# bendalab/audian

Hardware: AMD Instinct MI355X
Metric: Msamples/s spectrogram+bandpass, 64ch x 96kHz (higher is better)
Workload: dtype f32 I/O, f64 IIR state; 1 GPU; BASELINE configs[2]: synthetic 64 ch/GPU x 600 s x 96 kHz float32; bandpass 300-3000 Hz order 2 -> spectrogram nfft 2048 hop 1024 + envelope 20 Hz; channels_per_gpu=64, frames=57600000, spectrogram_frames=56250, parallelism=channel shard x1, streams=one compute stream, envelope_forward=state checkpoints, fused into the band-pass kernel, envelope_buffer=best of 4 allocations by memset time (hipdsp_malloc_probed), spectrogram=FFT waves inside the forward sweep (filtered tiles from LDS)

## Files before the change

### audian_amd/csrc/sos.hip

```cpp
#include "sos_device.h"
#include <cmath>
#include <vector>

namespace {
template <int S>
__global__ __launch_bounds__(64 * WPB) void sos_scan_kernel(const SosPlanDev *__restrict__ P0, SeqArgs a)
{
    constexpr int D = 2 * S;
    __shared__ float4 lds_all[WPB][64 * 8];
    const int wave = __builtin_amdgcn_readfirstlane(threadIdx.x >> 6);
    float4 *lds = lds_all[wave];
    const int lane = threadIdx.x & 63;
    const long long unit = (long long)blockIdx.x * WPB + wave;
    if (unit >= a.units) return;
    const int seg = (int)(unit % a.n_seg);
    const long long ch = unit / a.n_seg;
    const float *in = a.in + ch * a.in_pitch;
    float *out = a.out + ch * a.out_pitch;

    const long long lo = (long long)seg * a.seg_len;
    long long hi = lo + a.seg_len;
    if (hi > a.N) hi = a.N;
    long long start = lo - P0->warm;
    if (start < 0) start = 0;
// ... 260 lines not shown
    constexpr int D = 2 * SE;
    double *ckpt = ckpt_all + (long long)blockIdx.x * ckpt_pitch;
    flood_channel(flood, blockIdx.x);
    {
        __shared__ int any_bad;
        if (threadIdx.x == 0) any_bad = 0;
        __syncthreads();
        for (long long j = first_seg + threadIdx.x; j < n_seg; j += blockDim.x) {
            const double *e = ckpt + (j + 1 < n_seg ? (j + 1) * seg_tiles : n_tiles) * D;
            bool bad = false;
#pragma unroll
            for (int r = 0; r < D; r++) bad = bad || !(fabs(e[r]) <= 1.7976931348623157e308);
            if (bad) atomicOr(&any_bad, 1);
        }
        __syncthreads();
        if (any_bad && threadIdx.x == 0) ckpt[n_tiles * D] = __builtin_nan("");
        __syncthreads();
    }
    double AT[D][D];
#pragma unroll
    for (int r = 0; r < D; r++)
#pragma unroll
        for (int c = 0; c < D; c++) AT[r][c] = P0->AT[r * D + c];
    const long long warm_tiles = P0->warm / TILE;
    const long long terms = (warm_tiles + seg_tiles - 1) / seg_tiles + 1;
    const long long steps = seg_tiles <= warm_tiles ? seg_tiles : 0;
    for (long long k_hi = n_seg - 1; k_hi >= first_seg + 1; k_hi -= blockDim.x) {
        const long long k = k_hi - threadIdx.x;
        double S[D];
#pragma unroll
        for (int r = 0; r < D; r++) S[r] = 0.0;
        if (k >= first_seg + 1) {
            long long j = k - terms;
            if (j < first_seg) j = first_seg;
            for (; j < k; j++) {
                const double *e = ckpt + (j + 1) * seg_tiles * D;
                if (steps == 0) {
#pragma unroll
                    for (int r = 0; r < D; r++) S[r] = 0.0;
                }
                for (long long m = 0; m < steps; m++) {
                    double t[D];
#pragma unroll
                    for (int r = 0; r < D; r++) {
                        double acc = 0.0;
#pragma unroll
                        for (int c = 0; c < D; c++) acc = fma(AT[r][c], S[c], acc);
                        t[r] = acc;
                    }
#pragma unroll
                    for (int r = 0; r < D; r++) S[r] = t[r];
                }
#pragma unroll
                for (int r = 0; r < D; r++) S[r] += e[r];
            }
        }
        __syncthreads();
        if (k >= first_seg + 1) {
            const long long t0 = k * seg_tiles;
            long long cnt = (k == n_seg - 1) ? n_tiles - t0 : seg_tiles;
            if (cnt > warm_tiles + 1) cnt = warm_tiles + 1;
#pragma unroll
            for (int r = 0; r < D; r++) ckpt[t0 * D + r] = S[r];
            for (long long m = 1; m < cnt; m++) {
                double t[D];
#pragma unroll
                for (int r = 0; r < D; r++) {
                    double acc = 0.0;
#pragma unroll
                    for (int c = 0; c < D; c++) acc = fma(AT[r][c], S[c], acc);
                    t[r] = acc;
                }
#pragma unroll
                for (int r = 0; r < D; r++) { S[r] = t[r]; ckpt[(t0 + m) * D + r] += t[r]; }
            }
        }
        __syncthreads();
    }
}

int launch_env_fix(hipdsp_ctx *ctx, const SosPlanDev *edev, int SE, double *ckpt, long long ckpt_pitch, long long channels,
                   int n_seg, long long seg_len, long long n_tiles, const FloodArgs *flood, int first_seg = 0)
{
    if (n_seg <= 1) return HIPDSP_OK;
    dim3 grid((unsigned)channels), block(256);
    const long long seg_tiles = seg_len / TILE;
    FloodArgs fl;
    memset(&fl, 0, sizeof(fl));
    if (flood) fl = *flood;
    switch (SE) {
    case 1: hipLaunchKernelGGL((env_fix_kernel<1>), grid, block, 0, ctx->stream, edev, ckpt, ckpt_pitch, n_seg, seg_tiles, n_tiles, fl, first_seg); break;
    case 2: hipLaunchKernelGGL((env_fix_kernel<2>), grid, block, 0, ctx->stream, edev, ckpt, ckpt_pitch, n_seg, seg_tiles, n_tiles, fl, first_seg); break;
    case 3: hipLaunchKernelGGL((env_fix_kernel<3>), grid, block, 0, ctx->stream, edev, ckpt, ckpt_pitch, n_seg, seg_tiles, n_tiles, fl, first_seg); break;
    case 4: hipLaunchKernelGGL((env_fix_kernel<4>), grid, block, 0, ctx->stream, edev, ckpt, ckpt_pitch, n_seg, seg_tiles, n_tiles, fl, first_seg); break;
    default: return HIPDSP_OK;
    }
    return hd_launch_status("env_fix_kernel");
}

template <int SE, bool PREFETCH, bool PIN = true, bool TRACE = false, int WPB_ = WPB, bool REGW = (SE <= 2)>
__global__ __launch_bounds__(64 * WPB_, REGW ? 2 : 1) void env_bwd_kernel(const SosPlanDev *__restrict__ P0, BwdArgs a)
{
    long long tr_acc[6] = {0, 0, 0, 0, 0, 0};
    long long tr_last = TRACE ? clock64() : 0;
#define TRACE_AT(i)                                              \
    do {                                                         \
        if (TRACE) {                                             \
            const long long t_ = clock64();                      \
            tr_acc[(i)] += t_ - tr_last;                         \
            tr_last = t_;                                        \
        }                                                        \
    } while (0)
    constexpr int DE = 2 * SE;
    __shared__ float4 lds_all[WPB_][64 * 8];
    const int wave = __builtin_amdgcn_readfirstlane(threadIdx.x >> 6);
    float4 *lds = lds_all[wave];
    float *ldsf = reinterpret_cast<float *>(lds);
    const int lane = threadIdx.x & 63;
    const long long unit = (long long)blockIdx.x * WPB_ + wave;
    if (unit >= a.units) return;
    const int seg = (int)(unit % a.n_seg);
    const long long ch = unit / a.n_seg;
    const float *in = a.in + ch * a.in_pitch;
    float *out = a.out + ch * a.out_pitch;
    const double *ckpt = a.ckpt + ch * a.ckpt_pitch;
    const long long T = a.T;
    const int edge = a.edge;
    const long long trace_t0 = a.trace ? wall_clock64() : 0;
    const unsigned slot = wave_slot_of_simd();

    const long long rt_lo = (long long)seg * a.seg_tiles;
    long long rt_hi = rt_lo + a.seg_tiles;
    if (rt_hi > a.n_tiles) rt_hi = a.n_tiles;
    long long rt_start = rt_lo - a.warm_tiles;
    if (rt_start < 0) rt_start = 0;

    double cb_[DE];
#pragma unroll
    for (int r = 0; r < DE; r++) cb_[r] = 0.0;

    {
        double end_state[DE];
#pragma unroll
        for (int r = 0; r < DE; r++) end_state[r] = ckpt[a.n_tiles * DE + r];
        if (state_not_finite(end_state)) {
            long long p_lo = (a.n_tiles - rt_hi) * TILE, p_hi = (a.n_tiles - rt_lo) * TILE;
            if (p_lo < a.skip) p_lo = a.skip;
            if (p_hi > T) p_hi = T;
            for (long long p = p_lo + lane; p < p_hi; p += 64) out[p - a.skip] = __builtin_nanf("");
            return;
        }
    }

    v4f nx[8], nck[SE];
    bool pre = false;
    auto fetch = [&](long long tidx) {
        const long long tsrc = (a.debug & 2) ? 0 : tidx;
#pragma unroll
        for (int k = 0; k < 8; k++) nx[k] = asm_load16(in + tsrc * TILE + 256 * k + 4 * lane);
#pragma unroll
        for (int i = 0; i < SE; i++) nck[i] = asm_load16(ckpt + tidx * DE + 2 * i);
    };
    const long long top_full = T / TILE - 1;
    auto prefetchable = [&](long long tidx) {
        return tidx >= 0 && tidx <= top_full && tidx * TILE + TILE > a.skip && tidx * TILE >= a.lead;
    };
    const long long env_tile0 = a.env0 > 0 ? a.env0 - a.env0 % TILE : -1;
    if (PREFETCH) {
        const long long t0 = a.n_tiles - 1 - rt_start;
        pre = rt_start < rt_hi && prefetchable(t0);
        fetch(pre ? t0 : top_full);
        asm volatile("s_waitcnt vmcnt(0)" ::: "memory");
    }

    for (long long rt = rt_start; rt < rt_hi; rt++) {
        const long long tidx = a.n_tiles - 1 - rt;
        const long long tile = tidx * TILE;
        if (tile + TILE <= a.skip) break;
        if (a.fair) rotate_issue_priority(slot);
        double cfw_[DE];
        if (PREFETCH && pre) {
            if (a.rectify) {
#pragma unroll
                for (int k = 0; k < 8; k++) {
                    asm volatile("" : "+v"(nx[k]));
                    lds[lds_slot(8 * k + (lane >> 3), lane & 7)] =
                        make_float4(fabsf(nx[k].x), fabsf(nx[k].y), fabsf(nx[k].z), fabsf(nx[k].w));
                }
            } else {
#pragma unroll
                for (int k = 0; k < 8; k++) {
                    asm volatile("" : "+v"(nx[k]));
                    lds[lds_slot(8 * k + (lane >> 3), lane & 7)] = make_float4(nx[k].x, nx[k].y, nx[k].z, nx[k].w);
                }
            }
#pragma unroll
            for (int i = 0; i < SE; i++) {
                asm volatile("" : "+v"(nck[i]));
                const v2d d = __builtin_bit_cast(v2d, nck[i]);
                cfw_[2 * i] = d.x; cfw_[2 * i + 1] = d.y;
            }
            WAVE_SYNC();
        } else if (PREFETCH) {
            const long long lead = a.lead;
#pragma unroll 1
            for (int k = 0; k < 8; k++) {
                const long long p = tile + 256 * k + 4 * lane;
                auto at = [&](long long q) { return in + (q < lead ? lead : (q < T ? q : T - 1)); };
                auto ok = [&](long long q) { return q >= lead && q < T; };
                v4f t;
                t.x = asm_load4(at(p));
                t.y = asm_load4(at(p + 1));
                t.z = asm_load4(at(p + 2));
                t.w = asm_load4(at(p + 3));
                asm volatile("s_waitcnt vmcnt(0)" ::: "memory");
                asm volatile("" : "+v"(t));
                float4 v = make_float4(ok(p) ? t.x : 0.f, ok(p + 1) ? t.y : 0.f, ok(p + 2) ? t.z : 0.f,
                                       ok(p + 3) ? t.w : 0.f);
                if (a.rectify) v = make_float4(fabsf(v.x), fabsf(v.y), fabsf(v.z), fabsf(v.w));
                lds[lds_slot(8 * k + (lane >> 3), lane & 7)] = v;
            }
            v4f ck[SE];
#pragma unroll
            for (int i = 0; i < SE; i++) ck[i] = asm_load16(ckpt + tidx * DE + 2 * i);
            float ra = asm_load4(in + (T - 1));
            float rb = asm_load4(in + (lane < edge ? T - 2 - lane : T - 1));
            asm volatile("s_waitcnt vmcnt(0)" ::: "memory");
#pragma unroll
            for (int i = 0; i < SE; i++) {
                asm volatile("" : "+v"(ck[i]));
                const v2d d = __builtin_bit_cast(v2d, ck[i]);
                cfw_[2 * i] = d.x; cfw_[2 * i + 1] = d.y;
            }
            asm volatile("" : "+v"(ra));
            asm volatile("" : "+v"(rb));
            WAVE_SYNC();
            if (lane < edge) {
                const long long pj = T + lane;
                if (pj >= tile && pj < tile + TILE) {
                    if (a.rectify) { ra = fabsf(ra); rb = fabsf(rb); }
                    ldsf[lds_float_index((int)(pj - tile))] = 2.f * ra - rb;
                }
            }
        } else {
#pragma unroll
            for (int k = 0; k < 8; k++) {
                float4 v = load_four_from(in, tile + 256 * k + 4 * lane, a.lead, T);
                if (a.rectify) v = make_float4(fabsf(v.x), fabsf(v.y), fabsf(v.z), fabsf(v.w));
                lds[lds_slot(8 * k + (lane >> 3), lane & 7)] = v;
            }
#pragma unroll
            for (int r = 0; r < DE; r++) cfw_[r] = ckpt[tidx * DE + r];
        }
        WAVE_SYNC();
        if (!PREFETCH && tile + TILE > T) {
            if (lane < edge) {
                const long long pj = T + lane;
                if (pj >= tile && pj < tile + TILE) {
                    float ra = in[T - 1], rb = in[T - 2 - lane];
                    if (a.rectify) { ra = fabsf(ra); rb = fabsf(rb); }
                    ldsf[lds_float_index((int)(pj - tile))] = 2.f * ra - rb;
                }
            }
            WAVE_SYNC();
        }
        if (PREFETCH) WAVE_SYNC();
        if (tile == env_tile0) {
            (void)env_left_fill(ldsf, lane, (int)(a.env0 - tile), edge);
        }
        TRACE_AT(0);
        if (PREFETCH) {
            pre = rt + 1 < rt_hi && prefetchable(tidx - 1);
            fetch(pre ? tidx - 1 : top_full);
        }
        TRACE_AT(1);
#define CASC_S SE
#define CASC_PLAN() PLAN_OF(P0)
#define CASC_IN(v) (v)
#define CASC_PIN_GROUPS PIN
      if constexpr (REGW) {
#define CASC_CARRY_AFTER_F
        double w_[L];
#define CASC_CARRY cfw_
#define CASC_GAIN a.gain
#define CASC_NO_STORE
#define CASC_TAP(j, e, y) w_[(j)] = (y)
#include "sos_cascade.inc"
#undef CASC_TAP
#undef CASC_NO_STORE
#undef CASC_GAIN
#undef CASC_CARRY
        WAVE_SYNC();
        TRACE_AT(2);
        if (rt == 0) {
            int last = (int)(T + edge - 1 - tile);
            asm volatile("" : "+v"(last));
            const int lrow = last >> 5, lj = last & 31;
            double v0 = 0.0;
#pragma unroll
            for (int j = 0; j < L; j++) v0 = (j == lj) ? w_[j] : v0;
            v0 = __shfl(v0, lrow, 64);
#pragma unroll
            for (int j = 0; j < L; j++) w_[j] = (L * lane + j > last) ? v0 : w_[j];
            const SosPlanDev *P = PLAN_OF(P0);
#pragma unroll
            for (int r = 0; r < DE; r++) cb_[r] = P->zi[r] * v0;
        }
#define CASC_CARRY cb_
#define CASC_DOWN
#define CASC_X(j) w_[L - 1 - (j)]
#include "sos_cascade.inc"
#undef CASC_X
#undef CASC_DOWN
#undef CASC_CARRY
#undef CASC_CARRY_AFTER_F
      } else {
#define CASC_CARRY cfw_
#define CASC_GAIN a.gain
#include "sos_cascade.inc"
#undef CASC_GAIN
#undef CASC_CARRY
        WAVE_SYNC();
        TRACE_AT(2);
        if (rt == 0) {
            const int last = (int)(T + edge - 1 - tile);
            const float v0 = ldsf[lds_float_index(last)];
            WAVE_SYNC();
            for (int s2 = last + 1 + lane; s2 < TILE; s2 += 64) ldsf[lds_float_index(s2)] = v0;
            const SosPlanDev *P = PLAN_OF(P0);
#pragma unroll
            for (int r = 0; r < DE; r++) cb_[r] = P->zi[r] * (double)v0;
            WAVE_SYNC();
        }
#define CASC_CARRY cb_
#define CASC_REVERSED
#include "sos_cascade.inc"
#undef CASC_REVERSED
#undef CASC_CARRY
      }
#undef CASC_PIN_GROUPS
#undef CASC_S
#undef CASC_PLAN
#undef CASC_IN
        WAVE_SYNC();
        TRACE_AT(3);
        if (rt >= rt_lo) {
            if (tile >= a.skip && tile + TILE <= T) {
                v4f rows[8];
                tile_rows_from_lds(lds, lane, rows);
                if (a.clamp) {
                    const long long tdst = (a.debug & 1) ? a.skip : tile;
#pragma unroll
                    for (int k = 0; k < 8; k++) {
                        const v4f v = rows[k];
                        f4u t; t.x = max_zero(v.x); t.y = max_zero(v.y); t.z = max_zero(v.z); t.w = max_zero(v.w);
                        *reinterpret_cast<f4u *>(out + (tdst + 256 * k + 4 * lane - a.skip)) = t;
                    }
                } else {
#pragma unroll
                    for (int k = 0; k < 8; k++) {
                        const v4f v = rows[k];
                        f4u t; t.x = v.x; t.y = v.y; t.z = v.z; t.w = v.w;
                        *reinterpret_cast<f4u *>(out + (tile + 256 * k + 4 * lane - a.skip)) = t;
                    }
                }
                TRACE_AT(4);
                if (PREFETCH) asm volatile("s_waitcnt vmcnt(7)" ::: "memory");
            } else {
#pragma unroll
                for (int k = 0; k < 8; k++) {
                    float4 v = lds[lds_slot(8 * k + (lane >> 3), lane & 7)];
                    if (a.clamp) {
                        v.x = fmaxf(v.x, 0.f); v.y = fmaxf(v.y, 0.f); v.z = fmaxf(v.z, 0.f); v.w = fmaxf(v.w, 0.f);
                    }
                    store_four(out, tile + 256 * k + 4 * lane, v, a.skip, T, a.skip);
                }
                if (PREFETCH) asm volatile("s_waitcnt vmcnt(0)" ::: "memory");
            }
        } else if (PREFETCH) {
            asm volatile("s_waitcnt vmcnt(0)" ::: "memory");
        }
        WAVE_SYNC();
        TRACE_AT(5);
    }
#undef TRACE_AT
    if (a.trace && lane == 0 && unit < a.trace_rows) {
        unsigned hw;
        asm volatile("s_getreg_b32 %0, hwreg(HW_REG_HW_ID)" : "=s"(hw));
        long long *tr = a.trace + 9 * unit;
        tr[0] = trace_t0;
        tr[1] = wall_clock64();
        tr[2] = hw;
#pragma unroll
        for (int i = 0; i < 6; i++) tr[3 + i] = tr_acc[i];
    }
}

__global__ __launch_bounds__(256) void odd_ext_kernel(const float *__restrict__ x, long long x_pitch, long long T, int edge, int rectify,
                                                      float *__restrict__ out, long long out_pitch)
{
    const long long ch = blockIdx.y;
    const float *xc = x + ch * x_pitch;
    float *oc = out + ch * out_pitch;
    const long long N = T + 2LL * edge;
    auto r = [&](long long k) { const float v = xc[k]; return rectify ? fabsf(v) : v; };
    const long long i = 4 * ((long long)blockIdx.x * 256 + threadIdx.x);
    if (i >= N) return;
    if (i >= edge && i + 4 <= edge + T) {
        f4u v = *reinterpret_cast<const f4u *>(xc + (i - edge));
        if (rectify) { v.x = fabsf(v.x); v.y = fabsf(v.y); v.z = fabsf(v.z); v.w = fabsf(v.w); }
        *reinterpret_cast<f4u *>(oc + i) = v;
        return;
    }
    for (long long j = i; j < i + 4 && j < N; j++) {
        float v;
        if (j < edge) v = 2.f * r(0) - r(edge - j);
        else if (j < edge + T) v = r(j - edge);
        else v = 2.f * r(T - 1) - r(T - 2 - (j - edge - T));
        oc[j] = v;
    }
}

__global__ __launch_bounds__(256) void flip_kernel(const float *__restrict__ x, long long x_pitch, long long N, long long first, long long n,
                                                   int clamp, float *__restrict__ y, long long y_pitch)
{
    const long long ch = blockIdx.y;
    const float *xc = x + ch * x_pitch;
    float *yc = y + ch * y_pitch;
    auto cl = [&](float v) { return (clamp && v < 0.f) ? 0.f : v; };
    const long long i = 4 * ((long long)blockIdx.x * 256 + threadIdx.x);
    if (i >= n) return;
    if (i + 4 <= n) {
        const f4u v = *reinterpret_cast<const f4u *>(xc + (N - 1 - (first + i) - 3));
        f4u o; o.x = cl(v.w); o.y = cl(v.z); o.z = cl(v.y); o.w = cl(v.x);
        *reinterpret_cast<f4u *>(yc + i) = o;
        return;
    }
    for (long long j = i; j < n; j++) yc[j] = cl(xc[N - 1 - (first + j)]);
}

__global__ void first_sample_kernel(const float *__restrict__ x, long long x_pitch, long long channels, float *__restrict__ ref)
{
    const long long c = (long long)blockIdx.x * blockDim.x + threadIdx.x;
    if (c < channels) ref[c] = x[c * x_pitch];
}

__global__ __launch_bounds__(256) void copy_skip_kernel(const float *__restrict__ x, long long x_pitch, float *__restrict__ y,
                                                        long long y_pitch, long long n, long long skip)
{
    const long long ch = blockIdx.y;
    const float *xi = x + ch * x_pitch + skip;
    float *yo = y + ch * y_pitch;
    const long long n4 = n / 4;
    const long long i = (long long)blockIdx.x * 256 + threadIdx.x;
    if (i < n4) {
        *reinterpret_cast<f4u *>(yo + 4 * i) = *reinterpret_cast<const f4u *>(xi + 4 * i);
    } else if (i == n4) {
        for (long long k = 4 * n4; k < n; k++) yo[k] = xi[k];
    }
}

int launch_scan(hipdsp_ctx *ctx, const SosPlanDev *dev, int S, SeqArgs a, long long channels, long long warm)
{
    if (a.gain == 0.0) a.gain = 1.0;
    plan_segments(ctx, a.N, channels, warm, &a.seg_len, &a.n_seg, -1);
    a.units = channels * a.n_seg;
    long long blocks = (a.units + WPB - 1) / WPB;
// ... 418 lines not shown
```

### audian_amd/csrc/sos_cascade.inc

```
#ifndef CASC_PIN_GROUPS
#define CASC_PIN_GROUPS false
#define CASC_PIN_DEFAULTED
#endif
#ifndef CASC_STAMP
#define CASC_STAMP(n)
#define CASC_STAMP_DEFAULTED
#endif
#ifndef CASC_UNIT_OK
#define CASC_UNIT_OK true
#define CASC_UNIT_DEFAULTED
#endif
#ifdef CASC_REVERSED
#define CASC_ROW (63 - lane)
#define CASC_Q(q) (7 - (q))
#define CASC_E(k) (3 - (k))
#elif defined(CASC_DOWN)
#define CASC_ROW lane
#define CASC_Q(q) (7 - (q))
#define CASC_E(k) (3 - (k))
#else
#define CASC_ROW lane
#define CASC_Q(q) (q)
#define CASC_E(k) (k)
#endif
#ifdef CASC_DOWN
#define CASC_SHIFT1(x) casc_wave_shl1(x)
#define CASC_SHIFT32(x) casc_wave_shl32(x)
#define CASC_SHIFT(x, d) __shfl_down((x), (d), 64)
#define CASC_FED(d) (lane < 64 - (d))
#define CASC_HEAD (lane == 63)
#define CASC_LAST 0
#else
#define CASC_SHIFT1(x) casc_wave_shr1(x)
#define CASC_SHIFT32(x) casc_wave_shr32(x)
#define CASC_SHIFT(x, d) __shfl_up((x), (d), 64)
#define CASC_FED(d) (lane >= (d))
#define CASC_HEAD (lane == 0)
#define CASC_LAST 63
#endif
#ifdef CASC_X
#define CASC_XD(q, k) (CASC_X(4 * (q) + (k)))
#else
#define CASC_XD(q, k) ((double)CASC_IN(e[CASC_E(k)]))
#endif
{
    constexpr int CD = 2 * CASC_S;
        double f[CD];
#ifdef CASC_F_IN
#pragma unroll
        for (int r = 0; r < CD; r++) f[r] = CASC_F_IN[r];
#else
#pragma unroll
        for (int r = 0; r < CD; r++) f[r] = 0.0;
        constexpr int GQ = CD <= 2 ? 4 : (CD <= 4 ? 2 : 1);
#ifdef CASC_ROLLED_GROUPS
#pragma unroll 1
#else
#pragma unroll
#endif
        for (int q0 = 0; q0 < 8; q0 += GQ) {
            const SosPlanDev *P = CASC_PLAN();
            double gg[GQ * 4 * CD];
            if (CASC_PIN_GROUPS) {
#pragma unroll
                for (int i = 0; i < GQ * 4 * CD; i++) gg[i] = P->G[4 * q0 * CD + i];
#pragma unroll
                for (int i = 0; i < GQ * 4 * CD; i++) asm volatile("" : "+s"(gg[i]));
            }
#define CASC_G(q, k, r) ((CASC_PIN_GROUPS) ? gg[(4 * ((q) - q0) + (k)) * CD + (r)] : P->G[(4 * (q) + (k)) * CD + (r)])
#pragma unroll
            for (int q = q0; q < q0 + GQ; q++) {
#ifndef CASC_X
                const float4 v = lds[lds_slot(CASC_ROW, CASC_Q(q))];
                const float e[4] = {v.x, v.y, v.z, v.w};
#endif
#pragma unroll
                for (int k = 0; k < 4; k++) {
                    const double xd = CASC_XD(q, k);
#pragma unroll
                    for (int r = 0; r < CD; r++) f[r] = fma(CASC_G(q, k, r), xd, f[r]);
                }
            }
#undef CASC_G
#ifdef CASC_X
            __builtin_amdgcn_sched_barrier(0);
#endif
        }
#ifdef CASC_GAIN
#pragma unroll
        for (int r = 0; r < CD; r++) f[r] *= (CASC_GAIN);
#endif
#endif
        CASC_STAMP(0);
        {
#ifdef CASC_CARRY_AFTER_F
#pragma unroll
            for (int r = 0; r < CD; r++) asm volatile("" : "+v"(f[r]), "+v"(CASC_CARRY[r]));
#endif
            const SosPlanDev *P = CASC_PLAN();
            double t[CD];
#pragma unroll
            for (int r = 0; r < CD; r++) {
                double acc = 0.0;
#pragma unroll
                for (int c = 0; c < CD; c++)
                    if (c / 2 <= r / 2) acc = fma(P->M[r * CD + c], CASC_CARRY[c], acc);
                t[r] = acc;
            }
#pragma unroll
            for (int r = 0; r < CD; r++) f[r] += CASC_HEAD ? t[r] : 0.0;
        }
        constexpr int GK = CD <= 2 ? 6 : (CD <= 4 ? 2 : 1);
#pragma unroll
        for (int k0 = 0; k0 < 6; k0 += GK) {
            const SosPlanDev *P = CASC_PLAN();
            double mm[GK * CD * CD];
            if (CASC_PIN_GROUPS) {
#pragma unroll
                for (int i = 0; i < GK * CD * CD; i++) mm[i] = P->M[k0 * CD * CD + i];
#pragma unroll
                for (int i = 0; i < GK * CD * CD; i++)
                    if ((i % CD) / 2 <= ((i / CD) % CD) / 2) asm volatile("" : "+s"(mm[i]));
            }
#define CASC_M(k, r, c) ((CASC_PIN_GROUPS) ? mm[((k) - k0) * CD * CD + (r) * CD + (c)] : P->M[(k) * CD * CD + (r) * CD + (c)])
#pragma unroll
            for (int k = k0; k < k0 + GK; k++) {
                const int d = 1 << k;
                double q[CD];
#pragma unroll
                for (int c = 0; c < CD; c++) {
                    if (k == 0) {
                        q[c] = CASC_SHIFT1(f[c]);
                    } else if (k == 5) {
                        q[c] = CASC_SHIFT32(f[c]);
                    } else {
                        q[c] = CASC_SHIFT(f[c], d);
                    }
                }
                if (k == 0 || k == 5 || CASC_FED(d)) {
#pragma unroll
                    for (int r = 0; r < CD; r++) {
                        double acc = f[r];
#pragma unroll
                        for (int c = 0; c < CD; c++)
                            if (c / 2 <= r / 2) acc = fma(CASC_M(k, r, c), q[c], acc);
                        f[r] = acc;
                    }
                }
            }
#undef CASC_M
        }
        CASC_STAMP(1);
#ifdef CASC_NO_OUTPUT
#pragma unroll
        for (int r = 0; r < CD; r++) CASC_CARRY[r] = __shfl(f[r], CASC_LAST, 64);
#else
        double z[CD];
#pragma unroll
        for (int r = 0; r < CD; r++) {
            const double s = CASC_SHIFT1(f[r]);
            z[r] = CASC_HEAD ? CASC_CARRY[r] : s;
        }
#pragma unroll
        for (int r = 0; r < CD; r++) CASC_CARRY[r] = __shfl(f[r], CASC_LAST, 64);

        {
            const SosPlanDev *P = CASC_PLAN();
            double cf[CASC_S][5];
#pragma unroll
            for (int s = 0; s < CASC_S; s++)
#pragma unroll
                for (int k = 0; k < 5; k++) cf[s][k] = P->coef[s][k];
#ifdef CASC_GAIN
#pragma unroll
            for (int k = 0; k < 3; k++) cf[0][k] *= (CASC_GAIN);
#endif
#define CASC_PHASE3(UNIT)                                                                         \
            _Pragma("unroll")                                                                      \
            for (int q = 0; q < 8; q++) {                                                          \
                CASC_PHASE3_LOAD(q)                                                                \
                _Pragma("unroll")                                                                  \
                for (int k = 0; k < 4; k++) {                                                      \
                    double cur = CASC_XD(q, k);                                                    \
                    _Pragma("unroll")                                                              \
                    for (int s = 0; s < CASC_S; s++) {                                             \
                        if ((UNIT) && s > 0) {                                                     \
                            const double y = cur + z[2 * s];                                       \
                            z[2 * s] = fma(-cf[s][3], y, fma(cf[s][1], cur, z[2 * s + 1]));        \
                            z[2 * s + 1] = fma(-cf[s][4], y, cur);                                 \
                            cur = y;                                                               \
                        } else {                                                                   \
                            const double y = fma(cf[s][0], cur, z[2 * s]);                         \
                            z[2 * s] = fma(-cf[s][3], y, fma(cf[s][1], cur, z[2 * s + 1]));        \
                            z[2 * s + 1] = fma(-cf[s][4], y, cf[s][2] * cur);                      \
                            cur = y;                                                               \
                        }                                                                          \
                    }                                                                              \
                    CASC_PHASE3_OUT(q, k)                                                          \
                }                                                                                  \
                CASC_PHASE3_STORE(q)                                                               \
            }
#ifdef CASC_X
#define CASC_PHASE3_LOAD(q) float e[4] = {0.f, 0.f, 0.f, 0.f};
#else
#define CASC_PHASE3_LOAD(q) const float4 v = lds[lds_slot(CASC_ROW, CASC_Q(q))]; float e[4] = {v.x, v.y, v.z, v.w};
#endif
#ifndef CASC_NO_STORE
#define CASC_PHASE3_SET(k) e[CASC_E(k)] = (float)cur;
#define CASC_PHASE3_STORE(q) lds[lds_slot(CASC_ROW, CASC_Q(q))] = make_float4(e[0], e[1], e[2], e[3]);
#else
#define CASC_PHASE3_SET(k)
#define CASC_PHASE3_STORE(q)
#endif
#ifdef CASC_TAP
#define CASC_PHASE3_OUT(q, k) CASC_PHASE3_SET(k) CASC_TAP((4 * (q) + (k)), e[CASC_E(k)], cur);
#else
#define CASC_PHASE3_OUT(q, k) CASC_PHASE3_SET(k)
#endif
            if (CASC_S > 1 && (CASC_UNIT_OK) && P->unit_tail != 0) {
                CASC_PHASE3(true)
            } else {
                CASC_PHASE3(false)
            }
#undef CASC_PHASE3
#undef CASC_PHASE3_LOAD
#undef CASC_PHASE3_SET
#undef CASC_PHASE3_STORE
#undef CASC_PHASE3_OUT
        }
        CASC_STAMP(2);
#endif
}
#ifdef CASC_STAMP_DEFAULTED
#undef CASC_STAMP
#undef CASC_STAMP_DEFAULTED
#endif
#ifdef CASC_UNIT_DEFAULTED
#undef CASC_UNIT_OK
#undef CASC_UNIT_DEFAULTED
#endif
#ifdef CASC_PIN_DEFAULTED
#undef CASC_PIN_GROUPS
#undef CASC_PIN_DEFAULTED
#endif
#undef CASC_ROW
#undef CASC_Q
#undef CASC_E
#undef CASC_SHIFT1
#undef CASC_SHIFT32
#undef CASC_SHIFT
#undef CASC_FED
#undef CASC_HEAD
#undef CASC_LAST
#undef CASC_XD
```

### audian_amd/csrc/sos_device.h

```cpp
#pragma once
#include "common.h"
#include "sos_plan.h"

struct hipdsp_sosplan {
    SosPlanDev *host;
    SosPlanDev *dev;
    hipEvent_t uploaded;
    bool valid;
};

struct FloodArgs {
    const unsigned char *flags;
    int n_seg;
    long long seg_len;
    float *y;
    long long y_pitch, T, skip;
    float *psd, *db;
    long long psd_pitch, n_valid;
    int F, nfft, hop;
    int frame_off;
};

int hd_launch_env_fix(hipdsp_ctx *ctx, const SosPlanDev *edev, int SE, double *ckpt, long long ckpt_pitch, long long channels,
                      int n_seg, long long seg_len, long long n_tiles, const FloodArgs *flood, int first_seg = 0);

struct BwdArgs {
    const float *in;
    float *out;
    const double *ckpt;
    long long in_pitch, out_pitch, ckpt_pitch;
    long long T, skip;
    long long n_tiles;
    long long seg_tiles, warm_tiles;
    int n_seg, edge, rectify, clamp;
    double gain;
    long long units;
    long long lead, env0;
    long long *trace;
    long long trace_rows;
    int debug;
    int fair;
};

namespace {


typedef float f4u __attribute__((ext_vector_type(4), aligned(4)));
typedef float f2u __attribute__((ext_vector_type(2), aligned(4)));

struct SeqArgs {
    const float *in;
    float *out;
    long long in_pitch, out_pitch;
    long long N;
    long long seg_len;
    int n_seg;
    long long skip;
    const float *zi_ref;
    long long zi_ref_pitch;
    double zi_scale;
    double gain;
    long long units;
    unsigned char *flags;
};

__device__ __forceinline__ long long opaque_zero()
{
    int z;
    asm volatile("s_mov_b32 %0, 0" : "=s"(z));
    return (long long)z;
}

__device__ __forceinline__ int lds_slot(int row, int q) { return row * 8 + (q ^ ((row & 7) ^ ((row >> 3) & 1))); }
__device__ __forceinline__ int lds_float_index(int s) { return lds_slot(s >> 5, (s & 31) >> 2) * 4 + (s & 3); }

__device__ __forceinline__ float4 load_four(const float *in, long long p, long long n)
{
    if (p + 4 <= n) {
        const f4u t = *reinterpret_cast<const f4u *>(in + p);
        return make_float4(t.x, t.y, t.z, t.w);
    }
    float4 v;
    v.x = p < n ? in[p] : 0.f;
    v.y = p + 1 < n ? in[p + 1] : 0.f;
    v.z = p + 2 < n ? in[p + 2] : 0.f;
    v.w = p + 3 < n ? in[p + 3] : 0.f;
    return v;
}

__device__ __forceinline__ float4 load_four_from(const float *in, long long p, long long first, long long n)
{
    if (p >= first) return load_four(in, p, n);
    float4 v;
    v.x = 0.f;
    v.y = (p + 1 >= first && p + 1 < n) ? in[p + 1] : 0.f;
    v.z = (p + 2 >= first && p + 2 < n) ? in[p + 2] : 0.f;
    v.w = (p + 3 >= first && p + 3 < n) ? in[p + 3] : 0.f;
    return v;
}

__device__ __forceinline__ void store_four(float *out, long long p, float4 v, long long lo, long long hi,
                                           long long shift)
{
    if (p >= lo && p + 4 <= hi) {
        f4u t; t.x = v.x; t.y = v.y; t.z = v.z; t.w = v.w;
        *reinterpret_cast<f4u *>(out + (p - shift)) = t;
    } else {
        const float e[4] = {v.x, v.y, v.z, v.w};
#pragma unroll
        for (int k = 0; k < 4; k++)
            if (p + k >= lo && p + k < hi) out[p + k - shift] = e[k];
    }
}

#define PLAN_OF(ptr) (reinterpret_cast<const SosPlanDev *>(reinterpret_cast<const char *>(ptr) + opaque_zero()))

__device__ __forceinline__ double casc_wave_shr1(double x)
{
    const long long b = __builtin_bit_cast(long long, x);
    const int lo = __builtin_amdgcn_update_dpp(0, (int)b, 0x138, 0xf, 0xf, true);
    const int hi = __builtin_amdgcn_update_dpp(0, (int)(b >> 32), 0x138, 0xf, 0xf, true);
    return __builtin_bit_cast(double, ((long long)hi << 32) | (unsigned int)lo);
}

__device__ __forceinline__ double casc_wave_shr32(double x)
{
    const long long b = __builtin_bit_cast(long long, x);
    const auto lo = __builtin_amdgcn_permlane32_swap(0, (int)b, false, false);
    const auto hi = __builtin_amdgcn_permlane32_swap(0, (int)(b >> 32), false, false);
    return __builtin_bit_cast(double, ((long long)hi[0] << 32) | (unsigned int)lo[0]);
}

__device__ __forceinline__ double casc_wave_shl1(double x)
{
    const long long b = __builtin_bit_cast(long long, x);
    const int lo = __builtin_amdgcn_update_dpp(0, (int)b, 0x130, 0xf, 0xf, true);
    const int hi = __builtin_amdgcn_update_dpp(0, (int)(b >> 32), 0x130, 0xf, 0xf, true);
    return __builtin_bit_cast(double, ((long long)hi << 32) | (unsigned int)lo);
}
__device__ __forceinline__ double casc_wave_shl32(double x)
{
    const long long b = __builtin_bit_cast(long long, x);
    const auto lo = __builtin_amdgcn_permlane32_swap((int)b, 0, false, false);
    const auto hi = __builtin_amdgcn_permlane32_swap((int)(b >> 32), 0, false, false);
    return __builtin_bit_cast(double, ((long long)hi[1] << 32) | (unsigned int)lo[1]);
}

#define WAVE_SYNC()                                          \
    do {                                                     \
        __builtin_amdgcn_fence(__ATOMIC_ACQ_REL, "wavefront"); \
        __builtin_amdgcn_wave_barrier();                     \
    } while (0)

constexpr int WPB = 4;

struct CkptArgs {
    const float *in;
    float *yf;
    double *ckpt;
    long long in_pitch, yf_pitch, ckpt_pitch;
    long long T, seg_len;
    int n_seg, edge, rectify;
    long long units;
    double gain;
    unsigned char *flags;
    long long lead;
    long long env0;
};

struct GridShift {
    long long lead, env0;
    int frame_off;
};
inline GridShift hd_grid_shift(long long spec_first, long long env_first, int hop, int edge, bool with_env)
{
    GridShift g;
    const long long step = hop > 0 ? hop : 128;
    g.lead = hop > 0 ? (step - spec_first % step) % step : 0;
    if (with_env && env_first + g.lead > 0) {
        for (int tries = 0; tries < 4; tries++) {
            const long long r = (env_first + g.lead) % TILE;
            if (r >= edge && r + edge < TILE) break;
            g.lead += step;
        }
    }
    g.env0 = with_env ? env_first + g.lead : 0;
    g.frame_off = hop > 0 ? (int)((spec_first + g.lead) / step) : 0;
    return g;
}

typedef float v4f __attribute__((ext_vector_type(4)));
__device__ __forceinline__ void tile_rows_from_lds(const float4 *lds, int lane, v4f (&v)[8])
{
#pragma unroll
    for (int k = 0; k < 8; k++) {
        const float4 t = lds[lds_slot(8 * k + (lane >> 3), lane & 7)];
        v[k] = (v4f){t.x, t.y, t.z, t.w};
    }
    asm volatile("" : "+v"(v[0]), "+v"(v[1]), "+v"(v[2]), "+v"(v[3]), "+v"(v[4]), "+v"(v[5]), "+v"(v[6]), "+v"(v[7]));
}
typedef double v2d __attribute__((ext_vector_type(2)));
__device__ __forceinline__ v4f asm_load16(const void *p)
{
    v4f r;
    asm volatile("global_load_dwordx4 %0, %1, off" : "=v"(r) : "v"(p) : "memory");
    return r;
}
__device__ __forceinline__ float asm_load4(const float *p)
{
    float r;
    asm volatile("global_load_dword %0, %1, off" : "=v"(r) : "v"(p) : "memory");
    return r;
}

__device__ __forceinline__ void rotate_issue_priority(unsigned slot)
{
    const unsigned p = (slot + (unsigned)(__builtin_readcyclecounter() >> 14)) & 3u;
    if (p == 0) __builtin_amdgcn_s_setprio(0);
    else if (p == 1) __builtin_amdgcn_s_setprio(1);
    else if (p == 2) __builtin_amdgcn_s_setprio(2);
    else __builtin_amdgcn_s_setprio(3);
}
__device__ __forceinline__ float max_zero(float x)
{
    float r;
    asm("v_max_f32_e32 %0, 0, %1" : "=v"(r) : "v"(x));
    return r;
}
__device__ __forceinline__ void set_issue_priority(int p)
{
    if (p == 0) __builtin_amdgcn_s_setprio(0);
    else if (p == 1) __builtin_amdgcn_s_setprio(1);
    else if (p == 2) __builtin_amdgcn_s_setprio(2);
    else __builtin_amdgcn_s_setprio(3);
}
__device__ __forceinline__ unsigned wave_slot_of_simd()
{
    unsigned hw;
    asm volatile("s_getreg_b32 %0, hwreg(HW_REG_HW_ID, 0, 4)" : "=s"(hw));
    return hw;
}

inline void hd_note_sweep(hipdsp_ctx *ctx, long long lead, long long env0, long long frames, long long channels, int SE)
{
    ctx->sweep_lead = lead; ctx->sweep_env0 = env0; ctx->sweep_frames = frames; ctx->sweep_channels = channels;
    ctx->sweep_sections = SE;
}

struct TileStates {
    long long n_tiles, ckpt_pitch;
    size_t bytes(long long channels) const { return sizeof(double) * (size_t)ckpt_pitch * (size_t)channels; }
};
inline TileStates hd_tile_states(long long T, int edge, int SE)
{
    const long long n_tiles = (T + edge + TILE - 1) / TILE;
    return TileStates{n_tiles, (n_tiles + 1) * 2 * SE};
}

__device__ __forceinline__ float env_left_fill(float *ldsf, int lane, int q, int edge)
{
    const float r0 = ldsf[lds_float_index(q)];
    const float e0 = 2.f * r0 - ldsf[lds_float_index(q + edge)];
    float ev = 0.f;
    if (lane < edge) ev = 2.f * r0 - ldsf[lds_float_index(q + edge - lane)];
    WAVE_SYNC();
    if (lane < edge) ldsf[lds_float_index(q - edge + lane)] = ev;
    for (int s2 = lane; s2 < q - edge; s2 += 64) ldsf[lds_float_index(s2)] = e0;
    WAVE_SYNC();
    return e0;
}


template <int D>
__device__ __forceinline__ bool state_not_finite(const double (&c)[D])
{
    bool bad = false;
#pragma unroll
    for (int r = 0; r < D; r++) bad = bad || !(fabs(c[r]) <= 1.7976931348623157e308);
    return bad;
}

__device__ void flood_channel(const FloodArgs &f, long long ch)
{
    __shared__ int first_bad;
    if (f.flags == nullptr || f.n_seg <= 1) return;
    if (threadIdx.x == 0) first_bad = 0x7fffffff;
    __syncthreads();
    const unsigned char *fl = f.flags + ch * f.n_seg;
    for (int s2 = threadIdx.x; s2 < f.n_seg - 1; s2 += blockDim.x)
        if (fl[s2]) atomicMin(&first_bad, s2);
    __syncthreads();
    const int s0 = first_bad;
    if (s0 == 0x7fffffff) return;
    const float nan_ = __builtin_nanf("");
    const long long n1 = (long long)(s0 + 1) * f.seg_len;
    if (f.y != nullptr) {
        float *yc = f.y + ch * f.y_pitch;
        for (long long p = (n1 > f.skip ? n1 : f.skip) + threadIdx.x; p < f.T; p += blockDim.x) yc[p - f.skip] = nan_;
    }
    if (f.psd != nullptr || f.db != nullptr) {
// ... 59 lines not shown
```

### audian_amd/csrc/sos_plan.h

```cpp
#pragma once
#include "common.h"

constexpr int L = 32;
constexpr int TILE = 64 * L;
constexpr int MAXS = HIPDSP_MAX_SECTIONS;
constexpr int MAXD = 2 * MAXS;

struct SosPlanDev {
    double coef[MAXS][5];
    double G[L * MAXD];
    double M[6 * MAXD * MAXD];
    double zi[MAXD];
    double AT[MAXD * MAXD];
    long long warm;
    int n_sections;
    int edge;
    int unit_tail;
};

int hd_fill_plan(SosPlanDev *p, const double *sos, int S);
void hd_plan_segments_occ(long long n_cus, int w_max, int per_simd, int max_segments, long long N, long long channels,
                          long long warm, long long *seg_len, int *n_seg);
```

### audian_amd/csrc/sos_plan.hip

```cpp
#include "sos_plan.h"
#include <cfloat>
#include <cmath>
#include <vector>

namespace {

typedef long double real;
#if !defined(__HIP_DEVICE_COMPILE__)
static_assert(LDBL_MANT_DIG >= 64, "the plan tables need a long double wider than float64 on the host");
#endif

struct Mat {
    int d;
    real v[MAXD][MAXD];
};

Mat mat_identity(int d)
{
    Mat m; m.d = d;
    for (int i = 0; i < MAXD; i++) for (int j = 0; j < MAXD; j++) m.v[i][j] = (i == j && i < d) ? 1.0L : 0.0L;
    return m;
}

Mat mat_mul(const Mat &a, const Mat &b)
{
    Mat m = mat_identity(a.d);
    for (int i = 0; i < a.d; i++)
        for (int j = 0; j < a.d; j++) {
            real s = 0.0L;
            for (int k = 0; k < a.d; k++) s += a.v[i][k] * b.v[k][j];
            m.v[i][j] = s;
        }
    return m;
}

double mat_norm_inf(const Mat &a)
{
    double n = 0.0;
    for (int i = 0; i < a.d; i++) {
        double s = 0.0;
        for (int j = 0; j < a.d; j++) s += (double)fabsl(a.v[i][j]);
        if (!(s <= n)) n = s;
    }
    return n;
}

void cascade_step(const double coef[MAXS][5], int S, real *z, real x)
{
    real cur = x;
    for (int s = 0; s < S; s++) {
        real y = coef[s][0] * cur + z[2 * s];
        z[2 * s] = coef[s][1] * cur - coef[s][3] * y + z[2 * s + 1];
        z[2 * s + 1] = coef[s][2] * cur - coef[s][4] * y;
        cur = y;
    }
}

int fill_plan(SosPlanDev *p, const double *sos, int S)
{
    memset(p, 0, sizeof(*p));
    p->n_sections = S;
    const int D = 2 * S;
    for (int s = 0; s < S; s++) {
        const double *c = sos + 6 * s;
        if (c[3] != 1.0) {
            hipdsp_set_error("sos[%d][3] (a0) must be 1, got %g", s, c[3]);
            return HIPDSP_ERR_INVALID;
        }
        for (int k = 0; k < 6; k++)
            if (!std::isfinite(c[k])) {
                hipdsp_set_error("sos[%d][%d] is not finite", s, k);
                return HIPDSP_ERR_INVALID;
            }
        p->coef[s][0] = c[0]; p->coef[s][1] = c[1]; p->coef[s][2] = c[2];
        p->coef[s][3] = c[4]; p->coef[s][4] = c[5];
    }
    p->unit_tail = S > 1 ? 1 : 0;
    for (int s = 1; s < S; s++)
        if (!(p->coef[s][0] == 1.0 && p->coef[s][2] == 1.0 && fabs(p->coef[s][1]) == 2.0)) p->unit_tail = 0;
    Mat A = mat_identity(D);
    real B[MAXD] = {0};
    for (int c = 0; c < D; c++) {
        real z[MAXD] = {0};
        z[c] = 1.0L;
        cascade_step(p->coef, S, z, 0.0L);
        for (int r = 0; r < D; r++) A.v[r][c] = z[r];
    }
    {
        real z[MAXD] = {0};
        cascade_step(p->coef, S, z, 1.0L);
        for (int r = 0; r < D; r++) B[r] = z[r];
    }
    {
        real g[MAXD];
        for (int r = 0; r < D; r++) g[r] = B[r];
        for (int j = L - 1; j >= 0; j--) {
            for (int r = 0; r < D; r++) p->G[j * D + r] = (double)g[r];
            real t[MAXD] = {0};
            for (int r = 0; r < D; r++)
                for (int c = 0; c < D; c++) t[r] += A.v[r][c] * g[c];
            for (int r = 0; r < D; r++) g[r] = t[r];
        }
    }
    Mat pw = A;
    for (int k = 0; k < 5; k++) pw = mat_mul(pw, pw);
    static_assert(L == 32, "plan assumes L == 32");
    for (int k = 0; k < 6; k++) {
        for (int r = 0; r < D; r++)
            for (int c = 0; c < D; c++) p->M[k * D * D + r * D + c] = (double)pw.v[r][c];
        pw = mat_mul(pw, pw);
    }
    for (int r = 0; r < D; r++)
        for (int c = 0; c < D; c++) p->AT[r * D + c] = (double)pw.v[r][c];
    const double tol = ldexp(1.0, -60);
    const int MAXBITS = 40;
    std::vector<Mat> pows;
    pows.push_back(pw);
    long long m = 1;
    int top = 0;
    while (!(mat_norm_inf(pows[top]) < tol) && top < MAXBITS) {
        pows.push_back(mat_mul(pows[top], pows[top]));
        top++;
        m <<= 1;
    }
    if (!(mat_norm_inf(pows[top]) < tol)) {
        m = 1LL << 50;
    } else if (top > 0) {
        Mat acc = mat_identity(D);
        long long q = 0;
        for (int k = top - 1; k >= 0; k--) {
            Mat cand = mat_mul(acc, pows[k]);
            if (!(mat_norm_inf(cand) < tol)) { acc = cand; q += 1LL << k; }
        }
        m = q + 1;
    }
    p->warm = m * TILE;
    double scale = 1.0;
    for (int s = 0; s < S; s++) {
        const double *c = sos + 6 * s;
        double b0 = c[0], b1 = c[1], b2 = c[2], a1 = c[4], a2 = c[5];
        double B0 = b1 - a1 * b0, B1 = b2 - a2 * b0;
        double m00 = 1.0 + a1, m01 = -1.0, m10 = a2, m11 = 1.0;
        double det = m00 * m11 - m01 * m10;
        p->zi[2 * s] = scale * (B0 * m11 - m01 * B1) / det;
        p->zi[2 * s + 1] = scale * (m00 * B1 - m10 * B0) / det;
        scale *= (c[0] + c[1] + c[2]) / (c[3] + c[4] + c[5]);
    }
    int nb = 0, na = 0;
    for (int s = 0; s < S; s++) {
        if (sos[6 * s + 2] == 0.0) nb++;
        if (sos[6 * s + 5] == 0.0) na++;
    }
    p->edge = 3 * (2 * S + 1 - (nb < na ? nb : na));
    return HIPDSP_OK;
}

double tile_step_cost(long long w, int w_max, int per_simd)
{
    if (per_simd > 0) {
        const long long sw = (w + per_simd - 1) / per_simd;
        return sw <= 1 ? 0.65 : 0.5 * (double)sw;
    }
    if (per_simd == -1) return 7.0 + 0.5625 * (double)w;
    if (per_simd == -2) return 1.4 + 0.9125 * (double)w;
    return (double)w_max * (1.0 + 0.25 * (1.0 - (double)w / (double)w_max));
}

void plan_segments_occ(long long n_cus, int w_max, int per_simd, int max_segments, long long N, long long channels,
                       long long warm, long long *seg_len, int *n_seg)
{
    if (n_cus < 1) n_cus = 1;
    if (w_max < 1) w_max = 1;
    long long max_seg = (N + TILE - 1) / TILE;
    if (warm >= (1LL << 40)) max_seg = 1;
    if (max_segments > 0 && max_seg > max_segments) max_seg = max_segments;
    if (max_seg > 65536) max_seg = 65536;
    if (max_seg < 1) max_seg = 1;
    const long long slots = n_cus * w_max;
    long long best_n = 1, best_len = (N + TILE - 1) / TILE * TILE;
    double best_cost = -1.0;
    auto consider = [&](long long n) {
        if (n < 1) n = 1;
        if (n > max_seg) n = max_seg;
        long long len = ((N + n - 1) / n + TILE - 1) / TILE * TILE;
        if (len < TILE) len = TILE;
        const long long cnt = (N + len - 1) / len;
        const long long units = channels * cnt;
        const double span = (double)(len + (cnt > 1 ? warm : 0));
        double cost;
        if (units <= slots) cost = span * tile_step_cost((units + n_cus - 1) / n_cus, w_max, per_simd);
        else cost = (double)((units + slots - 1) / slots) * span * tile_step_cost(w_max, w_max, per_simd);
        if (best_cost < 0 || cost < best_cost * (1.0 - 1e-9)) { best_cost = cost; best_n = cnt; best_len = len; }
    };
    for (int w = w_max; w >= 1; w--) consider(n_cus * w / channels);
    for (long long rounds = 2; rounds <= 64; rounds++) consider(rounds * slots / channels);
    for (int half = 1; half < 16; half++) consider((n_cus / channels) >> half);
    consider(1);
    *seg_len = best_len;
    *n_seg = (int)best_n;
}

}

int hd_fill_plan(SosPlanDev *p, const double *sos, int S) { return fill_plan(p, sos, S); }

void hd_plan_segments_occ(long long n_cus, int w_max, int per_simd, int max_segments, long long N, long long channels,
                          long long warm, long long *seg_len, int *n_seg)
{
    plan_segments_occ(n_cus, w_max, per_simd, max_segments, N, channels, warm, seg_len, n_seg);
}

extern "C" {

int hipdsp_sos_plan_host(const double *host_sos, int n_sections, int64_t *warmup, int *edge, double *zi)
{
    HD_REQUIRE(host_sos != nullptr, "host_sos is NULL");
    if (n_sections < 1 || n_sections > MAXS) {
        hipdsp_set_error("n_sections %d not in 1..%d", n_sections, MAXS);
        return HIPDSP_ERR_UNSUPPORTED;
    }
    SosPlanDev tmp;
    int rc = fill_plan(&tmp, host_sos, n_sections);
    if (rc != HIPDSP_OK) return rc;
    if (warmup) *warmup = tmp.warm;
    if (edge) *edge = tmp.edge;
    if (zi)
        for (int k = 0; k < 2 * n_sections; k++) zi[k] = tmp.zi[k];
    return HIPDSP_OK;
}

int hipdsp_sos_segments_host(int64_t n_cus, int waves_max, int per_simd, int max_segments, int64_t frames,
                             int64_t channels, int64_t warmup, int64_t *segment_frames, int *n_segments)
{
    HD_REQUIRE(n_cus >= 1 && waves_max >= 1 && per_simd >= -2 && frames >= 1 && channels >= 1 && warmup >= 0 &&
               max_segments >= 0, "bad argument");
    HD_REQUIRE(segment_frames != nullptr && n_segments != nullptr, "NULL output");
    long long len = 0;
    int n = 0;
    plan_segments_occ(n_cus, waves_max, per_simd, max_segments, frames, channels, warmup, &len, &n);
    *segment_frames = len;
    *n_segments = n;
    return HIPDSP_OK;
}

}
```

Before: 233,400 Msamples/s.

## Use DPP row scans with per-lane matrix powers for cross-lane cascade carry

Replaces the generic shuffle-based cross-lane prefix scan in the SOS cascade with DPP row-shift steps inside 16-lane rows. These are followed by two cross-row steps that use per-lane precomputed matrix powers (PW table), for the single-section register-window path. It also adds a reduce-only variant for state-only passes that reads lane 63 and applies the full-tile transition. The goal is to cut ds_bpermute/shuffle latency in the f64 lane scan. In exchange it adds a 64-entry matrix power table to the plan and extra VGPRs for the lane weights, which could lower occupancy.

```diff
diff --git a/audian_amd/csrc/sos.hip b/audian_amd/csrc/sos.hip
--- a/audian_amd/csrc/sos.hip
+++ b/audian_amd/csrc/sos.hip
@@ -436,6 +436,9 @@
         }
     }
 
+    CascLaneW<DE> lane_w_;
+    if constexpr (REGW && SE == 1) casc_lane_weights<DE>(P0, lane, lane_w_);
+
     v4f nx[8], nck[SE];
     bool pre = false;
     auto fetch = [&](long long tidx) {
@@ -564,6 +567,7 @@
 #define CASC_PIN_GROUPS PIN
       if constexpr (REGW) {
 #define CASC_CARRY_AFTER_F
+#define CASC_DPP_W lane_w_
         double w_[L];
 #define CASC_CARRY cfw_
 #define CASC_GAIN a.gain
@@ -597,6 +601,7 @@
 #undef CASC_X
 #undef CASC_DOWN
 #undef CASC_CARRY
+#undef CASC_DPP_W
 #undef CASC_CARRY_AFTER_F
       } else {
 #define CASC_CARRY cfw_
diff --git a/audian_amd/csrc/sos_cascade.inc b/audian_amd/csrc/sos_cascade.inc
--- a/audian_amd/csrc/sos_cascade.inc
+++ b/audian_amd/csrc/sos_cascade.inc
@@ -92,7 +92,12 @@
 #endif
 #endif
         CASC_STAMP(0);
-        {
+#if defined(CASC_NO_OUTPUT) && !defined(CASC_DOWN) && !defined(HIPDSP_AB_NO_END_STATE_SUM)
+        constexpr bool casc_reduce = (CD <= 4);
+#else
+        constexpr bool casc_reduce = false;
+#endif
+        if constexpr (!casc_reduce) {
 #ifdef CASC_CARRY_AFTER_F
 #pragma unroll
             for (int r = 0; r < CD; r++) asm volatile("" : "+v"(f[r]), "+v"(CASC_CARRY[r]));
@@ -110,6 +115,116 @@
 #pragma unroll
             for (int r = 0; r < CD; r++) f[r] += CASC_HEAD ? t[r] : 0.0;
         }
+#if defined(CASC_DPP_W) && !defined(HIPDSP_AB_NO_LANE_SCAN)
+        constexpr bool casc_dpp = (CD == 2);
+#else
+        constexpr bool casc_dpp = false;
+#endif
+        if constexpr (casc_reduce) {
+        constexpr int GK = CD <= 2 ? 6 : 2;
+#pragma unroll
+        for (int k0 = 0; k0 < 6; k0 += GK) {
+            const SosPlanDev *P = CASC_PLAN();
+            double mm[GK * CD * CD];
+            if (CASC_PIN_GROUPS) {
+#pragma unroll
+                for (int i = 0; i < GK * CD * CD; i++) mm[i] = P->M[k0 * CD * CD + i];
+#pragma unroll
+                for (int i = 0; i < GK * CD * CD; i++)
+                    if ((i % CD) / 2 <= ((i / CD) % CD) / 2) asm volatile("" : "+s"(mm[i]));
+            }
+#define CASC_M(k, r, c) ((CASC_PIN_GROUPS) ? mm[((k) - k0) * CD * CD + (r) * CD + (c)] : P->M[(k) * CD * CD + (r) * CD + (c)])
+#pragma unroll
+            for (int k = k0; k < k0 + GK; k++) {
+                double q[CD];
+#pragma unroll
+                for (int c = 0; c < CD; c++) q[c] = casc_tree_shift(f[c], k);
+#pragma unroll
+                for (int r = 0; r < CD; r++) {
+                    double acc = f[r];
+#pragma unroll
+                    for (int c = 0; c < CD; c++)
+                        if (c / 2 <= r / 2) acc = fma(CASC_M(k, r, c), q[c], acc);
+                    f[r] = acc;
+                }
+            }
+#undef CASC_M
+        }
+        } else if constexpr (casc_dpp) {
+#ifdef CASC_DPP_W
+        {
+            const SosPlanDev *P = CASC_PLAN();
+            double mm[4 * CD * CD];
+#pragma unroll
+            for (int i = 0; i < 4 * CD * CD; i++) mm[i] = P->M[i];
+            if (CASC_PIN_GROUPS) {
+#pragma unroll
+                for (int i = 0; i < 4 * CD * CD; i++) asm volatile("" : "+s"(mm[i]));
+            }
+#define CASC_ROW_STEP(k, CTRL)                                                                     \
+            {                                                                                      \
+                double q[CD];                                                                      \
+                _Pragma("unroll")                                                                  \
+                for (int c = 0; c < CD; c++) q[c] = casc_dpp_f64<CTRL, 0xf>(f[c]);                 \
+                _Pragma("unroll")                                                                  \
+                for (int r = 0; r < CD; r++) {                                                     \
+                    double acc = f[r];                                                             \
+                    _Pragma("unroll")                                                              \
+                    for (int c = 0; c < CD; c++) acc = fma(mm[(k) * CD * CD + r * CD + c], q[c], acc); \
+                    f[r] = acc;                                                                    \
+                }                                                                                  \
+            }
+#define CASC_CROSS_STEP(W, Q)                                                                      \
+            _Pragma("unroll")                                                                      \
+            for (int r = 0; r < CD; r++) {                                                         \
+                double acc = f[r];                                                                 \
+                _Pragma("unroll")                                                                  \
+                for (int c = 0; c < CD; c++) acc = fma((W)[r * CD + c], (Q)[c], acc);              \
+                f[r] = acc;                                                                        \
+            }
+#ifdef CASC_DOWN
+            CASC_ROW_STEP(0, 0x101)
+            CASC_ROW_STEP(1, 0x102)
+            CASC_ROW_STEP(2, 0x104)
+            CASC_ROW_STEP(3, 0x108)
+            {
+                double q[CD];
+#pragma unroll
+                for (int c = 0; c < CD; c++) {
+                    const double s16 = casc_read_lane<16>(f[c]), s48 = casc_read_lane<48>(f[c]);
+                    q[c] = lane < 32 ? s16 : s48;
+                }
+                if ((lane & 16) == 0) { CASC_CROSS_STEP(CASC_DPP_W.dn1, q) }
+            }
+            {
+                double q[CD];
+#pragma unroll
+                for (int c = 0; c < CD; c++) q[c] = casc_read_lane<32>(f[c]);
+                if (lane < 32) { CASC_CROSS_STEP(CASC_DPP_W.dn2, q) }
+            }
+#else
+            CASC_ROW_STEP(0, 0x111)
+            CASC_ROW_STEP(1, 0x112)
+            CASC_ROW_STEP(2, 0x114)
+            CASC_ROW_STEP(3, 0x118)
+            {
+                double q[CD];
+#pragma unroll
+                for (int c = 0; c < CD; c++) q[c] = casc_dpp_f64<0x142, 0xa>(f[c]);
+                CASC_CROSS_STEP(CASC_DPP_W.up1, q)
+            }
+            {
+                double q[CD];
+#pragma unroll
+                for (int c = 0; c < CD; c++) q[c] = casc_dpp_f64<0x143, 0xc>(f[c]);
+                CASC_CROSS_STEP(CASC_DPP_W.up2, q)
+            }
+#endif
+#undef CASC_ROW_STEP
+#undef CASC_CROSS_STEP
+        }
+#endif
+        } else {
         constexpr int GK = CD <= 2 ? 6 : (CD <= 4 ? 2 : 1);
 #pragma unroll
         for (int k0 = 0; k0 < 6; k0 += GK) {
@@ -150,10 +265,31 @@
             }
 #undef CASC_M
         }
+        }
+#define CASC_END_STATE(x) (casc_dpp ? casc_read_lane<CASC_LAST>(x) : __shfl((x), CASC_LAST, 64))
         CASC_STAMP(1);
 #ifdef CASC_NO_OUTPUT
-#pragma unroll
-        for (int r = 0; r < CD; r++) CASC_CARRY[r] = __shfl(f[r], CASC_LAST, 64);
+        if constexpr (casc_reduce) {
+            const SosPlanDev *P = CASC_PLAN();
+            double t[CD];
+#pragma unroll
+            for (int r = 0; r < CD; r++) {
+                double acc = casc_read_lane<63>(f[r]);
+                asm volatile("" : "+v"(acc));
+#pragma unroll
+                for (int c = 0; c < CD; c++)
+                    if (c / 2 <= r / 2) acc = fma(P->AT[r * CD + c], CASC_CARRY[c], acc);
+                t[r] = acc;
+            }
+#pragma unroll
+            for (int r = 0; r < CD; r++) CASC_CARRY[r] = t[r];
+        } else {
+#pragma unroll
+            for (int r = 0; r < CD; r++) {
+                CASC_CARRY[r] = CASC_END_STATE(f[r]);
+                if (casc_dpp) asm volatile("" : "+v"(CASC_CARRY[r]));
+            }
+        }
 #else
         double z[CD];
 #pragma unroll
@@ -162,7 +298,10 @@
             z[r] = CASC_HEAD ? CASC_CARRY[r] : s;
         }
 #pragma unroll
-        for (int r = 0; r < CD; r++) CASC_CARRY[r] = __shfl(f[r], CASC_LAST, 64);
+        for (int r = 0; r < CD; r++) {
+            CASC_CARRY[r] = CASC_END_STATE(f[r]);
+            if (casc_dpp) asm volatile("" : "+v"(CASC_CARRY[r]));
+        }
 
         {
             const SosPlanDev *P = CASC_PLAN();
@@ -252,4 +391,5 @@
 #undef CASC_FED
 #undef CASC_HEAD
 #undef CASC_LAST
+#undef CASC_END_STATE
 #undef CASC_XD
diff --git a/audian_amd/csrc/sos_device.h b/audian_amd/csrc/sos_device.h
--- a/audian_amd/csrc/sos_device.h
+++ b/audian_amd/csrc/sos_device.h
@@ -146,6 +146,52 @@
     return __builtin_bit_cast(double, ((long long)hi[1] << 32) | (unsigned int)lo[1]);
 }
 
+template <int CTRL, int ROW_MASK>
+__device__ __forceinline__ double casc_dpp_f64(double x)
+{
+    const long long b = __builtin_bit_cast(long long, x);
+    const int lo = __builtin_amdgcn_update_dpp(0, (int)b, CTRL, ROW_MASK, 0xf, true);
+    const int hi = __builtin_amdgcn_update_dpp(0, (int)(b >> 32), CTRL, ROW_MASK, 0xf, true);
+    return __builtin_bit_cast(double, ((long long)hi << 32) | (unsigned int)lo);
+}
+__device__ __forceinline__ double casc_tree_shift(double x, int k)
+{
+    switch (k) {
+    case 0: return casc_dpp_f64<0x111, 0xf>(x);
+    case 1: return casc_dpp_f64<0x112, 0xf>(x);
+    case 2: return casc_dpp_f64<0x114, 0xf>(x);
+    case 3: return casc_dpp_f64<0x118, 0xf>(x);
+    case 4: return casc_dpp_f64<0x142, 0xa>(x);
+    default: return casc_dpp_f64<0x143, 0xc>(x);
+    }
+}
+template <int LANE>
+__device__ __forceinline__ double casc_read_lane(double x)
+{
+    const long long b = __builtin_bit_cast(long long, x);
+    const int lo = __builtin_amdgcn_readlane((int)b, LANE), hi = __builtin_amdgcn_readlane((int)(b >> 32), LANE);
+    return __builtin_bit_cast(double, ((long long)hi << 32) | (unsigned int)lo);
+}
+template <int CD>
+struct CascLaneW {
+    double up1[CD * CD], up2[CD * CD], dn1[CD * CD], dn2[CD * CD];
+};
+template <int CD>
+__device__ __forceinline__ void casc_lane_weights(const SosPlanDev *P, int lane, CascLaneW<CD> &w)
+{
+    const int j = lane & 15;
+    const int ku1 = j + 1, ku2 = lane >= 32 ? lane - 31 : 1, kd1 = 16 - j, kd2 = lane < 32 ? 32 - lane : 1;
+#pragma unroll
+    for (int i = 0; i < CD * CD; i++) {
+        w.up1[i] = P->PW[(ku1 - 1) * CD * CD + i];
+        w.up2[i] = P->PW[(ku2 - 1) * CD * CD + i];
+        w.dn1[i] = P->PW[(kd1 - 1) * CD * CD + i];
+        w.dn2[i] = P->PW[(kd2 - 1) * CD * CD + i];
+    }
+#pragma unroll
+    for (int i = 0; i < CD * CD; i++) asm volatile("" : "+v"(w.up1[i]), "+v"(w.up2[i]), "+v"(w.dn1[i]), "+v"(w.dn2[i]));
+}
+
 #define WAVE_SYNC()                                          \
     do {                                                     \
         __builtin_amdgcn_fence(__ATOMIC_ACQ_REL, "wavefront"); \
diff --git a/audian_amd/csrc/sos_plan.h b/audian_amd/csrc/sos_plan.h
--- a/audian_amd/csrc/sos_plan.h
+++ b/audian_amd/csrc/sos_plan.h
@@ -5,6 +5,7 @@
 constexpr int TILE = 64 * L;
 constexpr int MAXS = HIPDSP_MAX_SECTIONS;
 constexpr int MAXD = 2 * MAXS;
+constexpr int PW_MAXD = 4;
 
 struct SosPlanDev {
     double coef[MAXS][5];
@@ -16,6 +17,7 @@
     int n_sections;
     int edge;
     int unit_tail;
+    double PW[64 * PW_MAXD * PW_MAXD];
 };
 
 int hd_fill_plan(SosPlanDev *p, const double *sos, int S);
diff --git a/audian_amd/csrc/sos_plan.hip b/audian_amd/csrc/sos_plan.hip
--- a/audian_amd/csrc/sos_plan.hip
+++ b/audian_amd/csrc/sos_plan.hip
@@ -105,11 +105,26 @@
     Mat pw = A;
     for (int k = 0; k < 5; k++) pw = mat_mul(pw, pw);
     static_assert(L == 32, "plan assumes L == 32");
+    Mat lane_pw[7];
     for (int k = 0; k < 6; k++) {
+        lane_pw[k] = pw;
         for (int r = 0; r < D; r++)
             for (int c = 0; c < D; c++) p->M[k * D * D + r * D + c] = (double)pw.v[r][c];
         pw = mat_mul(pw, pw);
     }
+    lane_pw[6] = pw;
+    if (D <= PW_MAXD)
+        for (int k = 1; k <= 64; k++) {
+            Mat acc = mat_identity(D);
+            bool first = true;
+            for (int b = 6; b >= 0; b--)
+                if (k >> b & 1) {
+                    acc = first ? lane_pw[b] : mat_mul(acc, lane_pw[b]);
+                    first = false;
+                }
+            for (int r = 0; r < D; r++)
+                for (int c = 0; c < D; c++) p->PW[(k - 1) * D * D + r * D + c] = (double)acc.v[r][c];
+        }
     for (int r = 0; r < D; r++)
         for (int c = 0; c < D; c++) p->AT[r * D + c] = (double)pw.v[r][c];
     const double tol = ldexp(1.0, -60);
```

After: 233,800 Msamples/s (median of 2 runs). No clear change (+0.2%).
